# sreeramkannan/Shannon

Measured on AMD Instinct MI355X. Metric: reads/sec k-mer->graph->path-decompose, 2x100bp k=25, higher is better.
Workload: dtype u64

## Files before the change

### shannon_amd/csrc/count_sk.hip

```cpp
#include "count_views.h"
#include <algorithm>
#include <cstring>
#include <cstdlib>

#define SK_BLK 256
#define SK_RCAP 3072
#define SK_CHECK 4
#define SK_FLUSH_AT (SK_RCAP - (SK_CHECK + 1) * SK_BLK)
#define SK_TILE 32768
#define SK_CAP 2048
#ifndef SK_SCAP
#define SK_SCAP 2048
#endif
#ifndef SK_STHREADS
#define SK_STHREADS 256
#endif
#ifndef SK_T1CAP
#define SK_T1CAP 1024
#endif
#ifndef SK_T2THREADS
#define SK_T2THREADS 256
#endif
#define SK_SPILL 1280
#define SK_EMPTY 0xFFFFFFFFFFFFFFFFULL
#define SK_REGIONS 256
#define SK_RSTRIDE 16
#define SK_RANK_MAX 512
#define SK_MIN_K 20

struct SkParams { int k, m, w, bits, b1, b2; };

struct __attribute__((aligned(16))) SkRec { uint64_t hi; uint32_t lo; uint32_t meta; };

#define sk_order shn_sk_order
#define sk_bucket shn_sk_bucket

__device__ __forceinline__ void sk_extract96(const uint64_t* __restrict__ w, uint32_t nw, uint32_t p, uint64_t& hi, uint32_t& lo) {
  const uint32_t wi = p >> 5, sh = (p & 31) * 2;
  const uint64_t a = w[wi], b = wi + 1 < nw ? w[wi + 1] : 0ULL, c = (sh && wi + 2 < nw) ? w[wi + 2] : 0ULL;
  hi = sh ? (a << sh) | (b >> (64 - sh)) : a;
  const uint64_t l = sh ? (b << sh) | (c >> (64 - sh)) : b;
  lo = (uint32_t)(l >> 32);
}
__device__ __forceinline__ uint64_t sk_window(uint64_t hi, uint32_t lo, int j, int k) {
  const int sh = 2 * j;
  const uint64_t v = sh ? (hi << sh) | (((uint64_t)lo << 32) >> (64 - sh)) : hi;
  return v >> (64 - 2 * k);
}

__device__ __forceinline__ uint32_t sk_slot_hash(uint64_t key) { return (uint32_t)shn_mix64(key ^ 0x9E3779B97F4A7C15ULL); }

template <bool CANON>
__global__ __launch_bounds__(SK_BLK) void sk_scan_kernel(ReadsView v, SkParams P, uint32_t max_len, SkRec* __restrict__ slots, uint32_t S,
                                                         uint8_t* __restrict__ cnt, SkRec* __restrict__ ovf, unsigned long long* __restrict__ ovf_cursor,
                                                         uint64_t ovf_cap) {
  extern __shared__ uint32_t sk_lds[];
  uint32_t* raw = sk_lds;
  uint32_t* suf = raw + P.w * SK_BLK;
  const int tid = threadIdx.x;
  const int k = P.k, m = P.m, w = P.w;
  const uint32_t mmask = m == 16 ? 0xFFFFFFFFu : ((1u << (2 * m)) - 1u);
  const uint64_t n_tiles = (v.n_reads + SK_BLK - 1) / SK_BLK;
  for (uint64_t tile = blockIdx.x; tile < n_tiles; tile += gridDim.x) {
    const uint64_t r = tile * SK_BLK + tid;
    if (r >= v.n_reads) continue;
    const uint32_t len = v.len ? v.len[r] : v.fixed_len;
    const uint64_t wb = v.woff ? v.woff[r] : r * v.wpr;
    const uint32_t nw = v.woff ? (uint32_t)(v.woff[r + 1] - v.woff[r]) : v.wpr;
    const uint64_t* rw = v.words + wb;
    SkRec* mine = slots + r * S;
    uint64_t cur = 0, curm = 0;
    uint32_t f = 0, rr = 0, pref = 0xFFFFFFFFu, run_ord = 0, nrec = 0;
    int lastN = -1, t = 0, p0 = 0;
    bool open = false;

    auto emit = [&](int a, int b, uint32_t ord) {
      SkRec rec;
      sk_extract96(rw, nw, (uint32_t)a, rec.hi, rec.lo);
      rec.meta = (uint32_t)(b - a + 1) | (sk_bucket(ord, P.bits) << 5);
      if (nrec < S) mine[nrec] = rec;
      else {
        const unsigned long long at = atomicAdd(ovf_cursor, 1ULL);
        if (at < ovf_cap) ovf[at] = rec;
      }
      nrec++;
    };

    const uint32_t stop = len < max_len ? len : max_len;
    for (uint32_t j = 0; j < stop; j++) {
      if ((j & 31) == 0) cur = rw[j >> 5];
      const uint32_t b = (uint32_t)(cur >> (62 - 2 * (j & 31))) & 3u;
      if (v.has_n) {
        if ((j & 63) == 0) curm = v.mask[wb / 2 + (j >> 6)];
        if ((curm >> (63 - (j & 63))) & 1ULL) lastN = (int)j;
      }
      f = ((f << 2) | b) & mmask;
      rr = (rr >> 2) | ((3u - b) << (2 * (m - 1)));
      if ((int)j < m - 1) continue;
      const int i = (int)j - m + 1;
      const uint32_t ord = sk_order(CANON ? (f < rr ? f : rr) : f);
      raw[t * SK_BLK + tid] = ord;
      pref = t == 0 ? ord : (ord < pref ? ord : pref);
      if (i >= w - 1) {
        uint32_t wmin = pref;
        if (t != w - 1) { const uint32_t sv = suf[(t + 1) * SK_BLK + tid]; wmin = sv < wmin ? sv : wmin; }
        const int p = i - w + 1;
        const bool valid = lastN < p;
        if (open && (!valid || wmin != run_ord || p - p0 >= w)) { emit(p0, p - 1, run_ord); open = false; }
        if (valid && !open) { open = true; p0 = p; run_ord = wmin; }
      }
      if (t == w - 1) {
        uint32_t sm = 0xFFFFFFFFu;
        for (int tt = w - 1; tt >= 0; tt--) { const uint32_t x = raw[tt * SK_BLK + tid]; sm = x < sm ? x : sm; suf[tt * SK_BLK + tid] = sm; }
        t = 0;
      } else t++;
    }
    if (open) emit(p0, (int)len - k, run_ord);
    cnt[r] = (uint8_t)(nrec < S ? nrec : S);
  }
}

__device__ __forceinline__ bool skr_item(const SkRec* __restrict__ recs, const uint8_t* __restrict__ cnt, uint32_t S, uint64_t g, uint32_t& meta) {
  if (cnt) { const uint64_t r = g / S; if ((uint32_t)(g - r * S) >= cnt[r]) return false; }
  meta = recs[g].meta;
  return cnt || meta != 0;
}
__global__ __launch_bounds__(SK_BLK) void skr_hist_kernel(const SkRec* __restrict__ recs, const uint8_t* __restrict__ cnt, uint32_t S,
                                                          const uint64_t* __restrict__ segoff, uint32_t n_seg, int shift, uint32_t nb,
                                                          uint32_t* __restrict__ hist) {
  extern __shared__ uint32_t skh[];
  for (uint32_t p = blockIdx.y; p < n_seg; p += gridDim.y) {
    const uint64_t s0 = segoff[p], s1 = segoff[p + 1];
    const uint64_t t0 = s0 + (uint64_t)blockIdx.x * SK_TILE;
    if (t0 >= s1) continue;
    const uint64_t t1 = min(t0 + (uint64_t)SK_TILE, s1);
    for (uint32_t i = threadIdx.x; i < nb; i += SK_BLK) skh[i] = 0;
    __syncthreads();
    for (uint64_t i = t0 + threadIdx.x; i < t1; i += SK_BLK) {
      uint32_t meta;
      if (skr_item(recs, cnt, S, i, meta)) atomicAdd(&skh[((meta >> 5) >> shift) & (nb - 1)], 1u);
    }
    __syncthreads();
    for (uint32_t i = threadIdx.x; i < nb; i += SK_BLK) if (skh[i]) atomicAdd(&hist[(uint64_t)p * nb + i], skh[i]);
    __syncthreads();
  }
}
__global__ __launch_bounds__(SK_BLK) void skr_scan_rows_kernel(const uint32_t* __restrict__ hist, uint32_t nb2, uint32_t* __restrict__ off,
                                                               uint32_t* __restrict__ cursor) {
  __shared__ uint32_t part[SK_BLK];
  const uint64_t row = (uint64_t)blockIdx.x * nb2;
  const uint32_t per = (nb2 + SK_BLK - 1) / SK_BLK;
  uint32_t s = 0;
  for (uint32_t j = 0; j < per; j++) { const uint32_t i = threadIdx.x * per + j; if (i < nb2) s += hist[row + i]; }
  part[threadIdx.x] = s;
  __syncthreads();
  if (threadIdx.x == 0) { uint32_t a = 0; for (int i = 0; i < SK_BLK; i++) { const uint32_t t = part[i]; part[i] = a; a += t; } }
  __syncthreads();
  uint32_t a = part[threadIdx.x];
  for (uint32_t j = 0; j < per; j++) {
    const uint32_t i = threadIdx.x * per + j;
    if (i < nb2) { off[row + i] = a; cursor[row + i] = a; a += hist[row + i]; }
  }
}
__global__ __launch_bounds__(SK_BLK) void skr_scatter_kernel(const SkRec* __restrict__ recs, const uint8_t* __restrict__ cnt, uint32_t S,
                                                             const uint64_t* __restrict__ segoff, uint32_t n_seg, int shift, uint32_t nb,
                                                             uint32_t* __restrict__ cursor, const uint64_t* __restrict__ out_seg, SkRec* __restrict__ out) {
  extern __shared__ uint32_t sks[];
  uint32_t* lh = sks;
  uint32_t* lbase = sks + nb;
  for (uint32_t p = blockIdx.y; p < n_seg; p += gridDim.y) {
    const uint64_t s0 = segoff[p], s1 = segoff[p + 1];
    const uint64_t t0 = s0 + (uint64_t)blockIdx.x * SK_TILE;
    if (t0 >= s1) continue;
    const uint64_t t1 = min(t0 + (uint64_t)SK_TILE, s1);
    const uint64_t o0 = out_seg ? out_seg[p] : s0;
    for (uint32_t i = threadIdx.x; i < nb; i += SK_BLK) lh[i] = 0;
    __syncthreads();
    for (uint64_t i = t0 + threadIdx.x; i < t1; i += SK_BLK) {
      uint32_t meta;
      if (skr_item(recs, cnt, S, i, meta)) atomicAdd(&lh[((meta >> 5) >> shift) & (nb - 1)], 1u);
    }
    __syncthreads();
    for (uint32_t i = threadIdx.x; i < nb; i += SK_BLK) {
      const uint32_t c = lh[i];
      if (c) lbase[i] = atomicAdd(&cursor[(uint64_t)p * nb + i], c);
      lh[i] = 0;
    }
    __syncthreads();
    for (uint64_t i = t0 + threadIdx.x; i < t1; i += SK_BLK) {
      uint32_t meta;
      if (!skr_item(recs, cnt, S, i, meta)) continue;
      const SkRec rec = recs[i];
      const uint32_t q = ((meta >> 5) >> shift) & (nb - 1);
      const uint32_t rank = atomicAdd(&lh[q], 1u);
      out[o0 + lbase[q] + rank] = rec;
    }
    __syncthreads();
  }
}

template <bool CANON>
__global__ __launch_bounds__(SK_BLK) void sk_buckets_kernel(const SkRec* __restrict__ recs, const uint64_t* __restrict__ off1,
                                                            const uint32_t* __restrict__ off2, const uint32_t* __restrict__ hist2, int b2, int k, int w,
                                                            uint64_t* __restrict__ pool_keys, uint32_t* __restrict__ pool_counts,
                                                            unsigned long long* __restrict__ pool_cursor, uint64_t pool_cap) {
  constexpr int FOLD_ROUNDS_ = 2;
  __shared__ unsigned long long tk[SK_CAP];
  __shared__ uint32_t tc[SK_CAP];
  __shared__ uint32_t lnew, lpos;
  __shared__ unsigned long long lbase;
  const uint32_t b = blockIdx.x;
  const uint32_t n = hist2[b];
  if (n == 0) return;
  const uint64_t s0 = off1[b >> b2] + off2[b];
  const int tid = threadIdx.x, lane = tid & 63, q = tid & 7, grp = tid >> 3;
  for (int i = tid; i < SK_CAP; i += SK_BLK) { tk[i] = SK_EMPTY; tc[i] = 0; }
  if (tid == 0) { lnew = 0; lpos = 0; }
  __syncthreads();
  const int iters = (w + 7) >> 3;

  auto spill = [&]() {
    const uint32_t nd = lnew;
    if (tid == 0) lbase = atomicAdd(pool_cursor, (unsigned long long)nd);
    __syncthreads();
    const unsigned long long base = lbase;
    const bool fits = base + nd <= pool_cap;
    for (int i = tid; i < SK_CAP; i += SK_BLK) {
      const unsigned long long key = tk[i];
      if (key != SK_EMPTY) {
        if (fits) { const uint32_t pos = atomicAdd(&lpos, 1u); pool_keys[base + pos] = key; pool_counts[base + pos] = tc[i]; }
        tk[i] = SK_EMPTY; tc[i] = 0;
      }
    }
    __syncthreads();
    if (tid == 0) { lnew = 0; lpos = 0; }
    __syncthreads();
  };

  for (uint32_t base = 0; base < n; base += SK_BLK / 8) {
    __syncthreads();
    const bool full = lnew > SK_SPILL;
    __syncthreads();
    if (full) spill();
    const uint32_t ri = base + grp;
    SkRec rec;
    rec.hi = 0; rec.lo = 0; rec.meta = 0;
    if (ri < n) rec = recs[s0 + ri];
    const int nwin = (int)(rec.meta & 31u);
    for (int it = 0; it < iters; it++) {
      const int j = q + 8 * it;
      bool active = j < nwin;
      unsigned long long key = 0;
      if (active) {
        key = sk_window(rec.hi, rec.lo, j, k);
        if (CANON) { const uint64_t rc = shn_revcomp(key, k); key = rc < key ? rc : key; }
      }
      uint32_t wgt = active ? 1u : 0u;
      bool elect = active;
#pragma unroll
      for (int round = 0; round < FOLD_ROUNDS_; round++) {
        const unsigned long long act = __ballot(elect);
        if (!act) break;
        const int leader = __ffsll((long long)act) - 1;
        const unsigned long long lk = __shfl(key, leader, 64);
        const bool same = elect && key == lk;
        const unsigned long long msk = __ballot(same);
        if (__popcll(msk) > 1) {
          if (lane == leader) wgt = (uint32_t)__popcll(msk); else if (same) active = false;
        }
        if (same) elect = false;
      }
      if (!active) continue;
      uint32_t slot = (uint32_t)(shn_mix64(key ^ 0x9E3779B97F4A7C15ULL)) & (SK_CAP - 1);
      for (int probe = 0; probe < SK_CAP; probe++) {
        const unsigned long long prev = atomicCAS(&tk[slot], SK_EMPTY, key);
        if (prev == SK_EMPTY) { atomicAdd(&lnew, 1u); atomicAdd(&tc[slot], wgt); break; }
        if (prev == key) { atomicAdd(&tc[slot], wgt); break; }
        slot = (slot + 1) & (SK_CAP - 1);
      }
    }
  }
  __syncthreads();
  if (lnew) spill();
}

template <bool CANON, int THREADS, int CAP, int FOLD_ROUNDS_>
__global__ __launch_bounds__(THREADS) void sk_buckets_sorted_kernel(const SkRec* __restrict__ recs, const uint64_t* __restrict__ off1,
                                                                    const uint32_t* __restrict__ off2, const uint32_t* __restrict__ hist2, int b2, int k, int w,
                                                                    const uint32_t* __restrict__ list, uint32_t* __restrict__ defer, int defer_cursor,
                                                                    uint64_t* __restrict__ pool_keys, uint32_t* __restrict__ pool_counts,
                                                                    unsigned long long* __restrict__ cursors, uint64_t region_cap,
                                                                    unsigned long long* __restrict__ rcur,
                                                                    uint64_t* __restrict__ run_off, uint32_t* __restrict__ ndist) {
  extern __shared__ unsigned long long skb_lds[];
  unsigned long long* tk = skb_lds;
  uint32_t* tc = (uint32_t*)(tk + CAP);
  uint16_t* idx = (uint16_t*)(tc + CAP);
  __shared__ uint32_t lnew, lover, lpos;
  __shared__ unsigned long long lbase;
  const uint32_t b = list ? list[blockIdx.x] : blockIdx.x;
  const uint32_t n = hist2[b];
  const int tid = threadIdx.x, lane = tid & 63, q = tid & 7, grp = tid >> 3;
  if (n == 0) { if (tid == 0) { ndist[b] = 0; run_off[b] = 0; } return; }
  const uint64_t s0 = off1[b >> b2] + off2[b];
  const int iters = (w + 7) >> 3;
  const uint32_t limit = (uint32_t)(CAP - (THREADS / 8) * w - 64);

  auto pass = [&](uint32_t cls, int sbits) {
    for (int i = tid; i < CAP; i += THREADS) { tk[i] = SK_EMPTY; tc[i] = 0; }
    if (tid == 0) { lnew = 0; lover = 0; }
    __syncthreads();
    for (uint32_t base = 0; base < n; base += THREADS / 8) {
      __syncthreads();
      const bool full = lnew > limit;
      __syncthreads();
      if (full) { if (tid == 0) lover = 1; break; }
      const uint32_t ri = base + grp;
      SkRec rec;
      rec.hi = 0; rec.lo = 0; rec.meta = 0;
      if (ri < n) rec = recs[s0 + ri];
      const int nwin = (int)(rec.meta & 31u);
      for (int it = 0; it < iters; it++) {
        const int j = q + 8 * it;
        bool active = j < nwin;
        unsigned long long key = 0;
        if (active) {
          key = sk_window(rec.hi, rec.lo, j, k);
          if (CANON) { const uint64_t rc = shn_revcomp(key, k); key = rc < key ? rc : key; }
          if (sbits && (uint32_t)(key >> (2 * k - sbits)) != cls) active = false;
        }
        uint32_t wgt = active ? 1u : 0u;
        bool elect = active;
#pragma unroll
        for (int round = 0; round < FOLD_ROUNDS_; round++) {
          const unsigned long long act = __ballot(elect);
          if (!act) break;
          const int leader = __ffsll((long long)act) - 1;
          const unsigned long long lk = __shfl(key, leader, 64);
          const bool same = elect && key == lk;
          const unsigned long long msk = __ballot(same);
          if (__popcll(msk) > 1) {
            if (lane == leader) wgt = (uint32_t)__popcll(msk); else if (same) active = false;
          }
          if (same) elect = false;
        }
        if (!active) continue;
        uint32_t slot = sk_slot_hash(key) & (CAP - 1);
        for (int probe = 0; probe < CAP; probe++) {
          const unsigned long long prev = atomicCAS(&tk[slot], SK_EMPTY, key);
          if (prev == SK_EMPTY) { atomicAdd(&lnew, 1u); atomicAdd(&tc[slot], wgt); break; }
          if (prev == key) { atomicAdd(&tc[slot], wgt); break; }
          slot = (slot + 1) & (CAP - 1);
        }
      }
    }
    __syncthreads();
  };
  auto output = [&](uint64_t at) {
    const uint32_t nd = lnew;
    if (tid == 0) lpos = 0;
    __syncthreads();
    if (nd <= SK_RANK_MAX) {
      unsigned long long* dk = (unsigned long long*)idx;
      uint32_t* dc = (uint32_t*)(dk + SK_RANK_MAX);
      for (int i = tid; i < CAP; i += THREADS) {
        const unsigned long long key = tk[i];
        if (key != SK_EMPTY) { const uint32_t e = atomicAdd(&lpos, 1u); dk[e] = key; dc[e] = tc[i]; }
      }
      __syncthreads();
      for (uint32_t e = tid; e < nd; e += THREADS) {
        const unsigned long long key = dk[e];
        uint32_t r = 0;
        for (uint32_t j = 0; j < nd; j++) r += dk[j] < key ? 1u : 0u;
        pool_keys[at + r] = key; pool_counts[at + r] = dc[e];
      }
      __syncthreads();
      return;
    }
    for (int i = tid; i < CAP; i += THREADS) if (tk[i] != SK_EMPTY) idx[atomicAdd(&lpos, 1u)] = (uint16_t)i;
    uint32_t m2 = 1;
    while (m2 < nd) m2 <<= 1;
    __syncthreads();
    for (uint32_t i = nd + tid; i < m2; i += THREADS) idx[i] = 0xFFFFu;
    __syncthreads();
    for (uint32_t kk = 2; kk <= m2; kk <<= 1) {
      for (uint32_t j = kk >> 1; j > 0; j >>= 1) {
        for (uint32_t i = tid; i < m2; i += THREADS) {
          const uint32_t x = i ^ j;
          if (x > i) {
            const uint16_t ia = idx[i], ib = idx[x];
            const unsigned long long ka = ia == 0xFFFFu ? SK_EMPTY : tk[ia], kb = ib == 0xFFFFu ? SK_EMPTY : tk[ib];
            const bool asc = (i & kk) == 0;
            if ((ka > kb) == asc) { idx[i] = ib; idx[x] = ia; }
          }
        }
        __syncthreads();
      }
    }
    for (uint32_t i = tid; i < nd; i += THREADS) { const uint16_t ii = idx[i]; pool_keys[at + i] = tk[ii]; pool_counts[at + i] = tc[ii]; }
    __syncthreads();
  };

  int sbits = 0;
  uint32_t total = 0;
  for (;;) {
    total = 0;
    bool ok = true;
    for (uint32_t cls = 0; cls < (1u << sbits); cls++) {
      pass(cls, sbits);
      if (lover) { ok = false; break; }
      total += lnew;
      if (sbits == 0) break;
      __syncthreads();
    }
    if (ok) break;
    if (defer) {
      if (tid == 0) { const unsigned long long at = atomicAdd(&cursors[defer_cursor], 1ULL); defer[at] = b; ndist[b] = 0; run_off[b] = 0; }
      return;
    }
    sbits += 2;
    if (sbits > 16 || sbits > 2 * k) {
      if (tid == 0) { atomicAdd(&cursors[3], 1ULL); ndist[b] = 0; run_off[b] = 0; }
      return;
    }
    __syncthreads();
  }
  const uint32_t reg = b & (SK_REGIONS - 1);
  if (tid == 0) lbase = atomicAdd(&rcur[reg * SK_RSTRIDE], (unsigned long long)total);
  __syncthreads();
  const unsigned long long in_reg = lbase, base = (unsigned long long)reg * region_cap + in_reg;
  if (in_reg + total > region_cap) { if (tid == 0) { ndist[b] = 0; run_off[b] = 0; } return; }
  if (tid == 0) { ndist[b] = total; run_off[b] = base; }
  if (sbits == 0) { output(base); return; }
  uint64_t at = base;
  for (uint32_t cls = 0; cls < (1u << sbits); cls++) {
    pass(cls, sbits);
    const uint32_t nd = lnew;
    output(at);
    at += nd;
  }
}
__global__ __launch_bounds__(SK_BLK) void sk_gather_kernel(const uint64_t* __restrict__ pool_keys, const uint32_t* __restrict__ pool_counts,
                                                           const uint64_t* __restrict__ run_off, const uint32_t* __restrict__ ndist,
                                                           const uint64_t* __restrict__ boff, uint64_t n_buckets, uint64_t* __restrict__ keys,
                                                           uint32_t* __restrict__ counts) {
  const uint64_t b = ((uint64_t)blockIdx.x * SK_BLK + threadIdx.x) / SHN_WAVE;
  if (b >= n_buckets) return;
  const uint32_t lane = threadIdx.x & (SHN_WAVE - 1);
  const uint32_t nd = ndist[b];
  const uint64_t s0 = run_off[b], d0 = boff[b];
  for (uint32_t i = lane; i < nd; i += SHN_WAVE) { keys[d0 + i] = pool_keys[s0 + i]; counts[d0 + i] = pool_counts[s0 + i]; }
}
__global__ void sk_sum_counts_kernel(const uint32_t* __restrict__ c, uint64_t n, unsigned long long* __restrict__ out) {
  unsigned long long a = 0;
  for (uint64_t i = (uint64_t)blockIdx.x * blockDim.x + threadIdx.x; i < n; i += (uint64_t)gridDim.x * blockDim.x) a += c[i];
  for (int o = 32; o > 0; o >>= 1) a += __shfl_down(a, o, 64);
  if ((threadIdx.x & 63) == 0 && a) atomicAdd(out, a);
}

int shn_count_superkmers(shn_ctx* ctx, const std::vector<ReadsView>& views, uint64_t upper, int k1, int both_strands, shn_table** out, int* handled) {
  *handled = 0;
  const int mode = (int)shn_env_u64("SHN_COUNT_SK", 1);
  if (mode == 0 || k1 < SK_MIN_K || (k1 == 32 && !both_strands) || upper == 0) return SHN_OK;
  if (mode != 2 && upper < (1ULL << 22)) return SHN_OK;
  hipStream_t s = ctx->stream; shn_use_stream(s);
  SkParams P;
  P.k = k1;
  P.m = std::max(13, 2 * k1 - 48);
  P.w = k1 - P.m + 1;
  int bits = 6;
  while (bits < 22 && (upper >> bits) > 3500) bits++;
  bits = (int)shn_env_u64("SHN_COUNT_SK_BITS", (uint64_t)bits, 4, 22);
  P.bits = bits;
  P.b1 = (bits + 1) / 2;
  P.b2 = bits - P.b1;
  const uint32_t nb1 = 1u << P.b1, nb2 = 1u << P.b2;
  const uint64_t nbk = 1ULL << bits;
  struct ViewPlan { uint64_t slot0, read0; uint32_t S, max_len; };
  std::vector<ViewPlan> plan(views.size());
  uint64_t n_slots = 0, n_reads = 0;
  for (size_t i = 0; i < views.size(); i++) {
    const ReadsView& v = views[i];
    const double expect = 2.0 * v.wmax / (P.w + 1) + 1.0;
    uint32_t S = ((uint32_t)(expect * 1.35 + 1.999) + 3u) & ~3u;
    S = std::max<uint32_t>(1, std::min<uint32_t>(std::min<uint32_t>(S, 252), std::max<uint32_t>(v.wmax, 1)));
    S = (uint32_t)shn_env_u64("SHN_COUNT_SK_SLOTS", S, 1, 252);
    plan[i] = ViewPlan{n_slots, n_reads, S, v.wmax ? v.wmax + (uint32_t)k1 - 1 : 0u};
    if (v.wmax && v.n_reads) { n_slots += v.n_reads * S; n_reads += v.n_reads; }
  }
  const uint64_t ovf_cap = n_reads / 2 + 4096;
  int rc;
  void *p, *pslots, *pcnt;
  const size_t small = (size_t)nb1 * 4 * 3 + 64 + ((size_t)nb1 + 4) * 8 + nbk * 4 * 3 + 64 + (views.size() + 2) * 16;
  if ((rc = shn_ws(ctx)[22].get(small, &p))) return rc;
  if ((rc = shn_ws(ctx)[18].get((n_slots + ovf_cap + 2) * sizeof(SkRec), &pslots))) return rc;
  if ((rc = shn_ws(ctx)[23].get(n_reads + 64, &pcnt))) return rc;
  uint32_t* d_hist1 = (uint32_t*)p;
  uint32_t* d_offr1 = d_hist1 + nb1;
  uint32_t* d_cursor1 = d_offr1 + nb1;
  unsigned long long* d_cursors = (unsigned long long*)(d_cursor1 + nb1 + ((nb1 & 1) ? 1 : 0));
  uint64_t* d_seg = (uint64_t*)(d_cursors + 8);
  uint32_t* d_hist2 = (uint32_t*)(d_seg + nb1 + 4);
  uint32_t* d_off2 = d_hist2 + nbk;
  uint32_t* d_cursor2 = d_off2 + nbk;
  uint64_t* d_pairs = (uint64_t*)(d_cursor2 + nbk + (nbk & 1));
  SkRec* slots = (SkRec*)pslots;
  SkRec* ovf = slots + n_slots;
  uint8_t* d_cnt = (uint8_t*)pcnt;
  HIP_TRY(hipMemsetAsync(d_hist1, 0, (size_t)nb1 * 4, s));
  HIP_TRY(hipMemsetAsync(d_cursors, 0, 64, s));
  HIP_TRY(hipMemsetAsync(ovf, 0, ovf_cap * sizeof(SkRec), s));
  const size_t lds_scan = (size_t)2 * P.w * SK_BLK * 4;
  for (size_t i = 0; i < views.size(); i++) {
    const ReadsView& v = views[i];
    if (!v.wmax || !v.n_reads) continue;
    TimerRegion t(ctx, T_SK_EMIT);
    const uint32_t grid = (uint32_t)std::min<uint64_t>(cdiv(v.n_reads, SK_BLK), 1u << 20);
    if (both_strands) hipLaunchKernelGGL(sk_scan_kernel<true>, dim3(grid), dim3(SK_BLK), lds_scan, s, v, P, plan[i].max_len, slots + plan[i].slot0, plan[i].S,
                                         d_cnt + plan[i].read0, ovf, d_cursors, ovf_cap);
    else hipLaunchKernelGGL(sk_scan_kernel<false>, dim3(grid), dim3(SK_BLK), lds_scan, s, v, P, plan[i].max_len, slots + plan[i].slot0, plan[i].S,
                            d_cnt + plan[i].read0, ovf, d_cursors, ovf_cap);
  }
  std::vector<uint64_t> pairs(2 * (views.size() + 1), 0);
  for (size_t i = 0; i <= views.size(); i++) pairs[2 * i + 1] = i == views.size() ? ovf_cap : ((views[i].wmax && views[i].n_reads) ? views[i].n_reads * plan[i].S : 0);
  HIP_TRY(hipMemcpyAsync(d_pairs, pairs.data(), pairs.size() * 8, hipMemcpyHostToDevice, s));
  auto level1 = [&](bool scatter, SkRec* recsA) {
    for (size_t i = 0; i <= views.size(); i++) {
      const bool is_ovf = i == views.size();
      const uint64_t n = pairs[2 * i + 1];
      if (!n) continue;
      const SkRec* in = is_ovf ? ovf : slots + plan[i].slot0;
      const uint8_t* c = is_ovf ? nullptr : d_cnt + plan[i].read0;
      const uint32_t S = is_ovf ? 1u : plan[i].S;
      const uint32_t tiles = (uint32_t)std::max<uint64_t>(1, cdiv(n, SK_TILE));
      if (!scatter) hipLaunchKernelGGL(skr_hist_kernel, dim3(tiles, 1), dim3(SK_BLK), nb1 * 4, s, in, c, S, d_pairs + 2 * i, 1u, P.b2, nb1, d_hist1);
      else hipLaunchKernelGGL(skr_scatter_kernel, dim3(tiles, 1), dim3(SK_BLK), nb1 * 8, s, in, c, S, d_pairs + 2 * i, 1u, P.b2, nb1, d_cursor1,
                              (const uint64_t*)(d_cursors + 4), recsA);
    }
  };
  {
    TimerRegion t(ctx, T_SK_HIST);
    level1(false, nullptr);
  }
  std::vector<uint32_t> h1(nb1);
  unsigned long long ovf_used = 0;
  HIP_TRY(hipMemcpyAsync(h1.data(), d_hist1, (size_t)nb1 * 4, hipMemcpyDeviceToHost, s));
  HIP_TRY(hipMemcpyAsync(&ovf_used, d_cursors, 8, hipMemcpyDeviceToHost, s));
  HIP_TRY(hipStreamSynchronize(s));
  HIP_TRY(hipGetLastError());
  if (ovf_used > ovf_cap) return SHN_OK;
  std::vector<uint64_t> off1(nb1 + 1);
  std::vector<uint32_t> off1r(nb1);
  uint64_t NR = 0, max1 = 0;
  for (uint32_t i = 0; i < nb1; i++) { off1[i] = NR; NR += h1[i]; max1 = std::max<uint64_t>(max1, h1[i]); }
  off1[nb1] = NR;
  if (NR >= 0xFFFFFFFFULL) return SHN_OK;
  for (uint32_t i = 0; i < nb1; i++) off1r[i] = (uint32_t)off1[i];
  void* pa;
  if ((rc = shn_ws(ctx)[19].get((NR + 2) * sizeof(SkRec), &pa))) return rc;
  SkRec* recsA = (SkRec*)pa;
  SkRec* recsB = slots;
  HIP_TRY(hipMemcpyAsync(d_cursor1, off1r.data(), (size_t)nb1 * 4, hipMemcpyHostToDevice, s));
  HIP_TRY(hipMemcpyAsync(d_seg, off1.data(), (size_t)(nb1 + 1) * 8, hipMemcpyHostToDevice, s));
  HIP_TRY(hipMemsetAsync(d_hist2, 0, nbk * 4, s));
  HIP_TRY(hipStreamSynchronize(s));
  {
    TimerRegion t(ctx, T_SK_HIST);
    level1(true, recsA);
  }
  const uint32_t tiles = (uint32_t)std::max<uint64_t>(1, cdiv(max1, SK_TILE));
  {
    TimerRegion t(ctx, T_SK_HIST2);
    hipLaunchKernelGGL(skr_hist_kernel, dim3(tiles, nb1), dim3(SK_BLK), nb2 * 4, s, recsA, (const uint8_t*)nullptr, 1u, d_seg, nb1, 0, nb2, d_hist2);
  }
  hipLaunchKernelGGL(skr_scan_rows_kernel, dim3(nb1), dim3(SK_BLK), 0, s, d_hist2, nb2, d_off2, d_cursor2);
  {
    TimerRegion t(ctx, T_SK_SCATTER2);
    hipLaunchKernelGGL(skr_scatter_kernel, dim3(tiles, nb1), dim3(SK_BLK), nb2 * 8, s, recsA, (const uint8_t*)nullptr, 1u, d_seg, nb1, 0, nb2, d_cursor2,
                       (const uint64_t*)nullptr, recsB);
  }
  double ratio = ctx->sk_pool_ratio > 0 ? ctx->sk_pool_ratio * 1.05 : 0.125;
  ratio = shn_env_double("SHN_COUNT_SK_POOL", ratio);
  uint64_t cap = std::min<uint64_t>(upper, (uint64_t)((double)upper * ratio) + 4096);
  uint64_t np = 0;
  void *pk = nullptr, *pc = nullptr;
  bool sorted = shn_env_u64("SHN_COUNT_SK_LAYOUT", 1) != 0;
  if (sorted) {
    void* pr;
    if ((rc = shn_ws(ctx)[24].get(nbk * 20 + 64, &pr))) return rc;
    uint64_t* d_run_off = (uint64_t*)pr;
    uint32_t* d_ndist = (uint32_t*)(d_run_off + nbk);
    uint32_t* d_defer = d_ndist + nbk;
    uint32_t* d_defer2 = d_defer + nbk;
    constexpr int T1_CAP = SK_T1CAP, T2_CAP = SK_SCAP, BIG_T = 1024, BIG_CAP = 8192;
    const size_t lds_t1 = (size_t)T1_CAP * 12 + std::max<size_t>((size_t)T1_CAP * 2, (size_t)SK_RANK_MAX * 12),
                 lds_t2 = (size_t)T2_CAP * 12 + std::max<size_t>((size_t)T2_CAP * 2, (size_t)SK_RANK_MAX * 12), lds_big = (size_t)BIG_CAP * 14;
    HIP_TRY(hipFuncSetAttribute((const void*)sk_buckets_sorted_kernel<true, BIG_T, BIG_CAP, 2>, hipFuncAttributeMaxDynamicSharedMemorySize, (int)lds_big));
    HIP_TRY(hipFuncSetAttribute((const void*)sk_buckets_sorted_kernel<false, BIG_T, BIG_CAP, 2>, hipFuncAttributeMaxDynamicSharedMemorySize, (int)lds_big));
    unsigned long long cur[8] = {0, 0, 0, 0, 0, 0, 0, 0};
    void* prc;
    if ((rc = shn_ws(ctx)[29].get((size_t)SK_REGIONS * SK_RSTRIDE * 8, &prc))) return rc;
    unsigned long long* d_rcur = (unsigned long long*)prc;
    std::vector<unsigned long long> h_rcur((size_t)SK_REGIONS * SK_RSTRIDE);
    for (int attempt = 0; attempt < 3 && sorted; attempt++) {
      const uint64_t region_cap = cap / SK_REGIONS + 64;
      if ((rc = shn_ws(ctx)[20].get((region_cap * SK_REGIONS + 2) * 8, &pk))) return rc;
      if ((rc = shn_ws(ctx)[21].get((region_cap * SK_REGIONS + 2) * 4, &pc))) return rc;
      HIP_TRY(hipMemsetAsync(d_cursors + 1, 0, 56, s));
      HIP_TRY(hipMemsetAsync(d_rcur, 0, (size_t)SK_REGIONS * SK_RSTRIDE * 8, s));
      {
#define SK_LAUNCH(CANON_, T_, CAP_, FOLD_, GRID_, LDS_, LIST_, DEFER_, DCUR_) \
        hipLaunchKernelGGL((sk_buckets_sorted_kernel<CANON_, T_, CAP_, FOLD_>), dim3((uint32_t)(GRID_)), dim3(T_), LDS_, s, recsB, d_seg, d_off2, d_hist2, P.b2, k1, P.w, \
                           (const uint32_t*)(LIST_), (uint32_t*)(DEFER_), DCUR_, (uint64_t*)pk, (uint32_t*)pc, d_cursors, region_cap, d_rcur, d_run_off, d_ndist)
        { TimerRegion t(ctx, T_SK_BUCKETS);
          if (both_strands) SK_LAUNCH(true, SK_STHREADS, T1_CAP, 0, nbk, lds_t1, nullptr, d_defer, 2);
          else SK_LAUNCH(false, SK_STHREADS, T1_CAP, 0, nbk, lds_t1, nullptr, d_defer, 2); }
        HIP_TRY(hipMemcpyAsync(cur, d_cursors, 64, hipMemcpyDeviceToHost, s));
        HIP_TRY(hipStreamSynchronize(s));
        const unsigned long long n_t2 = cur[2];
        if (n_t2) {
          TimerRegion t2(ctx, T_SK_BUCKETS2);
          if (both_strands) SK_LAUNCH(true, SK_T2THREADS, T2_CAP, 0, n_t2, lds_t2, d_defer, d_defer2, 6);
          else SK_LAUNCH(false, SK_T2THREADS, T2_CAP, 0, n_t2, lds_t2, d_defer, d_defer2, 6);
          HIP_TRY(hipMemcpyAsync(cur, d_cursors, 64, hipMemcpyDeviceToHost, s));
          HIP_TRY(hipStreamSynchronize(s));
        }
        if (shn_env_set("SHN_COUNT_SK_DEBUG")) fprintf(stderr, "[sk] buckets %llu, %llu of them to 2,048 slots, %llu to 8,192; pool of %llu pairs in %d stretches\n", (unsigned long long)nbk, n_t2, cur[6], (unsigned long long)cap, SK_REGIONS);
        if (cur[6]) {
          TimerRegion tb(ctx, T_SK_BIG);
          if (both_strands) SK_LAUNCH(true, BIG_T, BIG_CAP, 2, cur[6], lds_big, d_defer2, nullptr, 2);
          else SK_LAUNCH(false, BIG_T, BIG_CAP, 2, cur[6], lds_big, d_defer2, nullptr, 2);
          HIP_TRY(hipMemcpyAsync(cur, d_cursors, 64, hipMemcpyDeviceToHost, s));
          HIP_TRY(hipStreamSynchronize(s));
        }
#undef SK_LAUNCH
      }
      HIP_TRY(hipGetLastError());
      if (cur[3]) { sorted = false; break; }
      HIP_TRY(hipMemcpyAsync(h_rcur.data(), d_rcur, h_rcur.size() * 8, hipMemcpyDeviceToHost, s));
      HIP_TRY(hipStreamSynchronize(s));
      unsigned long long fullest = 0;
      np = 0;
      for (int r_ = 0; r_ < SK_REGIONS; r_++) { const unsigned long long u = h_rcur[(size_t)r_ * SK_RSTRIDE]; np += u; fullest = std::max(fullest, u); }
      if (fullest <= region_cap) break;
      if (attempt == 2) return shn_fail(SHN_ERR_OVERFLOW, "shn_count_k1mers: the pair pool of the super-k-mer path stayed too small");
      cap = std::max<uint64_t>(np + np / 64 + 4096, (fullest + fullest / 64 + 64) * SK_REGIONS);
    }
    if (sorted) {
      if (!shn_env_set("SHN_COUNT_SK_POOL")) ctx->sk_pool_ratio = (double)np / (double)upper;
      shn_table* t = new shn_table();
      memset(t, 0, sizeof(*t));
      t->ctx = ctx; t->device = ctx->device; t->k = k1; t->canonical = both_strands ? 1 : 0; t->bits = bits; t->n_buckets = nbk;
      t->layout = 1; t->sk_m = P.m; t->n = np;
#define TRYT(x) do { hipError_t _e = (x); if (_e != hipSuccess) { shn_table_destroy(t); return shn_fail(SHN_ERR_HIP, std::string(#x) + ": " + hipGetErrorString(_e)); } } while (0)
      TRYT(shn_dev_malloc(&t->d_keys, (np + 1) * 8));
      TRYT(shn_dev_malloc(&t->d_counts, (np + 1) * 4));
      TRYT(shn_dev_malloc(&t->d_bucket_off, (nbk + 1) * 8));
      uint64_t D = 0;
      { TimerRegion tr(ctx, T_COMPACT);
        if ((rc = shn_device_scan_u32(ctx, d_ndist, nbk, t->d_bucket_off, &D))) { shn_table_destroy(t); return rc; }
        if (D != np) { shn_table_destroy(t); return shn_fail(SHN_ERR_OVERFLOW, "shn_count_k1mers: super-k-mer buckets and pool disagree"); }
        if (np) hipLaunchKernelGGL(sk_gather_kernel, dim3((uint32_t)cdiv(nbk * SHN_WAVE, SK_BLK)), dim3(SK_BLK), 0, s, (const uint64_t*)pk, (const uint32_t*)pc,
                                   (const uint64_t*)d_run_off, (const uint32_t*)d_ndist, (const uint64_t*)t->d_bucket_off, nbk, t->d_keys, t->d_counts);
        TRYT(hipMemsetAsync(d_cursors + 5, 0, 8, s));
        if (np) hipLaunchKernelGGL(sk_sum_counts_kernel, dim3(1024), dim3(256), 0, s, (const uint32_t*)t->d_counts, np, d_cursors + 5);
        unsigned long long tot = 0;
        TRYT(hipMemcpyAsync(&tot, d_cursors + 5, 8, hipMemcpyDeviceToHost, s));
        TRYT(hipStreamSynchronize(s));
        TRYT(hipGetLastError());
        t->total = tot;
      }
#undef TRYT
      *out = t;
      *handled = 1;
      return SHN_OK;
    }
  }
  for (int attempt = 0; attempt < 3; attempt++) {
    if ((rc = shn_ws(ctx)[20].get((cap + 2) * 8, &pk))) return rc;
    if ((rc = shn_ws(ctx)[21].get((cap + 2) * 4, &pc))) return rc;
    HIP_TRY(hipMemsetAsync(d_cursors + 1, 0, 8, s));
    {
      TimerRegion t(ctx, T_SK_BUCKETS);
      if (both_strands) hipLaunchKernelGGL(sk_buckets_kernel<true>, dim3((uint32_t)nbk), dim3(SK_BLK), 0, s, recsB, d_seg, d_off2, d_hist2, P.b2, k1, P.w,
                                           (uint64_t*)pk, (uint32_t*)pc, d_cursors + 1, cap);
      else hipLaunchKernelGGL(sk_buckets_kernel<false>, dim3((uint32_t)nbk), dim3(SK_BLK), 0, s, recsB, d_seg, d_off2, d_hist2, P.b2, k1, P.w,
                              (uint64_t*)pk, (uint32_t*)pc, d_cursors + 1, cap);
    }
    unsigned long long used = 0;
    HIP_TRY(hipMemcpyAsync(&used, d_cursors + 1, 8, hipMemcpyDeviceToHost, s));
    HIP_TRY(hipStreamSynchronize(s));
    HIP_TRY(hipGetLastError());
    np = used;
    if (np <= cap) break;
    if (attempt == 2) return shn_fail(SHN_ERR_OVERFLOW, "shn_count_k1mers: the pair pool of the super-k-mer path stayed too small");
    cap = std::min<uint64_t>(upper, np + np / 64 + 4096);
  }
  if (np >= 0xFFFFFFFFULL) return SHN_OK;
  rc = shn_table_from_pairs(ctx, pk, pc, np, k1, both_strands ? 1 : 0, out);
  if (rc) return rc;
  HIP_TRY(hipStreamSynchronize(s));
  *handled = 1;
  return SHN_OK;
}
```

Measured before the change: 66.75 million.

## Load-balance super-k-mer windows across threads and pre-route large buckets to deferred tiers

The bucket counting kernel now spreads windows evenly over threads. It stages one record per thread in LDS, takes a block prefix sum of window counts, and has each thread binary-search its start record. Before, each 8-thread group handled one record, which wasted lanes on short records. Buckets with more records than a threshold now skip straight to the deferred list, so they are not half-counted in the small table, and the next record is prefetched while the current round runs. The cost is extra syncs, a binary search, more LDS and a new routing parameter, plus a debug histogram.

```diff
diff --git a/shannon_amd/csrc/count_sk.hip b/shannon_amd/csrc/count_sk.hip
--- a/shannon_amd/csrc/count_sk.hip
+++ b/shannon_amd/csrc/count_sk.hip
@@ -26,6 +26,12 @@
 #define SK_REGIONS 256
 #define SK_RSTRIDE 16
 #define SK_RANK_MAX 512
+#ifndef SK_ROUTE1
+#define SK_ROUTE1 1536u
+#endif
+#ifndef SK_ROUTE2
+#define SK_ROUTE2 0xFFFFFFFFu
+#endif
 #define SK_MIN_K 20
 
 struct SkParams { int k, m, w, bits, b1, b2; };
@@ -287,45 +293,80 @@
 template <bool CANON, int THREADS, int CAP, int FOLD_ROUNDS_>
 __global__ __launch_bounds__(THREADS) void sk_buckets_sorted_kernel(const SkRec* __restrict__ recs, const uint64_t* __restrict__ off1,
                                                                     const uint32_t* __restrict__ off2, const uint32_t* __restrict__ hist2, int b2, int k, int w,
-                                                                    const uint32_t* __restrict__ list, uint32_t* __restrict__ defer, int defer_cursor,
+                                                                    const uint32_t* __restrict__ list, uint32_t* __restrict__ defer, int defer_cursor, uint32_t route,
                                                                     uint64_t* __restrict__ pool_keys, uint32_t* __restrict__ pool_counts,
                                                                     unsigned long long* __restrict__ cursors, uint64_t region_cap,
                                                                     unsigned long long* __restrict__ rcur,
                                                                     uint64_t* __restrict__ run_off, uint32_t* __restrict__ ndist) {
-  extern __shared__ unsigned long long skb_lds[];
+  static_assert(CAP > THREADS + 64 && THREADS % 64 == 0, "a round of THREADS windows must fit the table");
+  extern __shared__ __attribute__((aligned(16))) unsigned long long skb_lds[];
   unsigned long long* tk = skb_lds;
   uint32_t* tc = (uint32_t*)(tk + CAP);
   uint16_t* idx = (uint16_t*)(tc + CAP);
+  SkRec* stage = (SkRec*)idx;
+  uint32_t* wend = (uint32_t*)(stage + THREADS);
   __shared__ uint32_t lnew, lover, lpos;
+  __shared__ uint32_t wsum[THREADS / 64];
   __shared__ unsigned long long lbase;
   const uint32_t b = list ? list[blockIdx.x] : blockIdx.x;
   const uint32_t n = hist2[b];
-  const int tid = threadIdx.x, lane = tid & 63, q = tid & 7, grp = tid >> 3;
+  const uint64_t o1 = off1[b >> b2];
+  const uint32_t o2 = off2[b];
+  const int tid = threadIdx.x, lane = tid & 63;
   if (n == 0) { if (tid == 0) { ndist[b] = 0; run_off[b] = 0; } return; }
-  const uint64_t s0 = off1[b >> b2] + off2[b];
-  const int iters = (w + 7) >> 3;
-  const uint32_t limit = (uint32_t)(CAP - (THREADS / 8) * w - 64);
+  if (defer && n > route) {
+    if (tid == 0) { const unsigned long long at = atomicAdd(&cursors[defer_cursor], 1ULL); defer[at] = b; ndist[b] = 0; run_off[b] = 0; }
+    return;
+  }
+  const uint64_t s0 = o1 + o2;
+  const uint32_t limit = (uint32_t)(CAP - THREADS - 64);
 
   auto pass = [&](uint32_t cls, int sbits) {
+    SkRec nxt;
+    nxt.hi = 0; nxt.lo = 0; nxt.meta = 0;
+    if ((uint32_t)tid < n) nxt = recs[s0 + tid];
     for (int i = tid; i < CAP; i += THREADS) { tk[i] = SK_EMPTY; tc[i] = 0; }
     if (tid == 0) { lnew = 0; lover = 0; }
-    __syncthreads();
-    for (uint32_t base = 0; base < n; base += THREADS / 8) {
+    uint32_t bound = 0;
+    bool over = false;
+    for (uint32_t base = 0; base < n && !over; base += THREADS) {
+      const SkRec rec = nxt;
+      uint32_t inc = rec.meta & 31u;
+      for (int o = 1; o < 64; o <<= 1) { const uint32_t y = __shfl_up(inc, o, 64); if (lane >= o) inc += y; }
       __syncthreads();
-      const bool full = lnew > limit;
+      stage[tid] = rec;
+      if (lane == 63) wsum[tid >> 6] = inc;
       __syncthreads();
-      if (full) { if (tid == 0) lover = 1; break; }
-      const uint32_t ri = base + grp;
-      SkRec rec;
-      rec.hi = 0; rec.lo = 0; rec.meta = 0;
-      if (ri < n) rec = recs[s0 + ri];
-      const int nwin = (int)(rec.meta & 31u);
-      for (int it = 0; it < iters; it++) {
-        const int j = q + 8 * it;
-        bool active = j < nwin;
+      uint32_t pre = 0, W = 0;
+      for (int i = 0; i < THREADS / 64; i++) { const uint32_t x = wsum[i]; pre += i < (tid >> 6) ? x : 0u; W += x; }
+      wend[tid] = pre + inc;
+      nxt.hi = 0; nxt.lo = 0; nxt.meta = 0;
+      if (base + THREADS + (uint32_t)tid < n) nxt = recs[s0 + base + THREADS + tid];
+      __syncthreads();
+      const uint32_t c = (W + THREADS - 1) / THREADS;
+      const uint32_t g = (uint32_t)tid * c;
+      uint32_t r = 0;
+      if (g < W) {
+        uint32_t lo_ = 0, hi_ = THREADS - 1;
+        while (lo_ < hi_) { const uint32_t mid = (lo_ + hi_) >> 1; if (wend[mid] > g) hi_ = mid; else lo_ = mid + 1; }
+        r = lo_;
+      }
+      SkRec cur = stage[r];
+      uint32_t nwr = cur.meta & 31u;
+      uint32_t j = g < W ? g - (wend[r] - nwr) : 0u;
+      for (uint32_t i = 0; i < c; i++) {
+        if (bound > limit) {
+          __syncthreads();
+          bound = lnew;
+          __syncthreads();
+          if (bound > limit) { if (tid == 0) lover = 1; over = true; break; }
+        }
+        bound += THREADS;
+        bool active = g + i < W;
+        const bool mine = active;
         unsigned long long key = 0;
         if (active) {
-          key = sk_window(rec.hi, rec.lo, j, k);
+          key = sk_window(cur.hi, cur.lo, (int)j, k);
           if (CANON) { const uint64_t rc = shn_revcomp(key, k); key = rc < key ? rc : key; }
           if (sbits && (uint32_t)(key >> (2 * k - sbits)) != cls) active = false;
         }
@@ -344,13 +385,18 @@
           }
           if (same) elect = false;
         }
-        if (!active) continue;
-        uint32_t slot = sk_slot_hash(key) & (CAP - 1);
-        for (int probe = 0; probe < CAP; probe++) {
-          const unsigned long long prev = atomicCAS(&tk[slot], SK_EMPTY, key);
-          if (prev == SK_EMPTY) { atomicAdd(&lnew, 1u); atomicAdd(&tc[slot], wgt); break; }
-          if (prev == key) { atomicAdd(&tc[slot], wgt); break; }
-          slot = (slot + 1) & (CAP - 1);
+        if (active) {
+          uint32_t slot = sk_slot_hash(key) & (CAP - 1);
+          for (int probe = 0; probe < CAP; probe++) {
+            const unsigned long long prev = atomicCAS(&tk[slot], SK_EMPTY, key);
+            if (prev == SK_EMPTY) { atomicAdd(&lnew, 1u); atomicAdd(&tc[slot], wgt); break; }
+            if (prev == key) { atomicAdd(&tc[slot], wgt); break; }
+            slot = (slot + 1) & (CAP - 1);
+          }
+        }
+        if (mine && ++j == nwr && g + i + 1 < W) {
+          do { r++; cur = stage[r]; nwr = cur.meta & 31u; } while (nwr == 0 && r < THREADS - 1);
+          j = 0;
         }
       }
     }
@@ -593,8 +639,10 @@
     uint32_t* d_defer = d_ndist + nbk;
     uint32_t* d_defer2 = d_defer + nbk;
     constexpr int T1_CAP = SK_T1CAP, T2_CAP = SK_SCAP, BIG_T = 1024, BIG_CAP = 8192;
-    const size_t lds_t1 = (size_t)T1_CAP * 12 + std::max<size_t>((size_t)T1_CAP * 2, (size_t)SK_RANK_MAX * 12),
-                 lds_t2 = (size_t)T2_CAP * 12 + std::max<size_t>((size_t)T2_CAP * 2, (size_t)SK_RANK_MAX * 12), lds_big = (size_t)BIG_CAP * 14;
+    auto lds_of = [](size_t cap_, size_t threads) { return cap_ * 12 + std::max<size_t>(std::max<size_t>(cap_ * 2, (size_t)SK_RANK_MAX * 12), threads * 20); };
+    const size_t lds_t1 = lds_of(T1_CAP, SK_STHREADS), lds_t2 = lds_of(T2_CAP, SK_T2THREADS), lds_big = lds_of(BIG_CAP, BIG_T);
+    const bool sk_debug = shn_env_set("SHN_COUNT_SK_DEBUG");
+    const uint32_t route1 = sk_debug ? 0xFFFFFFFFu : SK_ROUTE1, route2 = sk_debug ? 0xFFFFFFFFu : SK_ROUTE2;
     HIP_TRY(hipFuncSetAttribute((const void*)sk_buckets_sorted_kernel<true, BIG_T, BIG_CAP, 2>, hipFuncAttributeMaxDynamicSharedMemorySize, (int)lds_big));
     HIP_TRY(hipFuncSetAttribute((const void*)sk_buckets_sorted_kernel<false, BIG_T, BIG_CAP, 2>, hipFuncAttributeMaxDynamicSharedMemorySize, (int)lds_big));
     unsigned long long cur[8] = {0, 0, 0, 0, 0, 0, 0, 0};
@@ -609,27 +657,44 @@
       HIP_TRY(hipMemsetAsync(d_cursors + 1, 0, 56, s));
       HIP_TRY(hipMemsetAsync(d_rcur, 0, (size_t)SK_REGIONS * SK_RSTRIDE * 8, s));
       {
-#define SK_LAUNCH(CANON_, T_, CAP_, FOLD_, GRID_, LDS_, LIST_, DEFER_, DCUR_) \
+#define SK_LAUNCH(CANON_, T_, CAP_, FOLD_, GRID_, LDS_, LIST_, DEFER_, DCUR_, ROUTE_) \
         hipLaunchKernelGGL((sk_buckets_sorted_kernel<CANON_, T_, CAP_, FOLD_>), dim3((uint32_t)(GRID_)), dim3(T_), LDS_, s, recsB, d_seg, d_off2, d_hist2, P.b2, k1, P.w, \
-                           (const uint32_t*)(LIST_), (uint32_t*)(DEFER_), DCUR_, (uint64_t*)pk, (uint32_t*)pc, d_cursors, region_cap, d_rcur, d_run_off, d_ndist)
+                           (const uint32_t*)(LIST_), (uint32_t*)(DEFER_), DCUR_, ROUTE_, (uint64_t*)pk, (uint32_t*)pc, d_cursors, region_cap, d_rcur, d_run_off, d_ndist)
         { TimerRegion t(ctx, T_SK_BUCKETS);
-          if (both_strands) SK_LAUNCH(true, SK_STHREADS, T1_CAP, 0, nbk, lds_t1, nullptr, d_defer, 2);
-          else SK_LAUNCH(false, SK_STHREADS, T1_CAP, 0, nbk, lds_t1, nullptr, d_defer, 2); }
+          if (both_strands) SK_LAUNCH(true, SK_STHREADS, T1_CAP, 0, nbk, lds_t1, nullptr, d_defer, 2, route1);
+          else SK_LAUNCH(false, SK_STHREADS, T1_CAP, 0, nbk, lds_t1, nullptr, d_defer, 2, route1); }
         HIP_TRY(hipMemcpyAsync(cur, d_cursors, 64, hipMemcpyDeviceToHost, s));
         HIP_TRY(hipStreamSynchronize(s));
         const unsigned long long n_t2 = cur[2];
         if (n_t2) {
           TimerRegion t2(ctx, T_SK_BUCKETS2);
-          if (both_strands) SK_LAUNCH(true, SK_T2THREADS, T2_CAP, 0, n_t2, lds_t2, d_defer, d_defer2, 6);
-          else SK_LAUNCH(false, SK_T2THREADS, T2_CAP, 0, n_t2, lds_t2, d_defer, d_defer2, 6);
+          if (both_strands) SK_LAUNCH(true, SK_T2THREADS, T2_CAP, 0, n_t2, lds_t2, d_defer, d_defer2, 6, route2);
+          else SK_LAUNCH(false, SK_T2THREADS, T2_CAP, 0, n_t2, lds_t2, d_defer, d_defer2, 6, route2);
           HIP_TRY(hipMemcpyAsync(cur, d_cursors, 64, hipMemcpyDeviceToHost, s));
           HIP_TRY(hipStreamSynchronize(s));
         }
-        if (shn_env_set("SHN_COUNT_SK_DEBUG")) fprintf(stderr, "[sk] buckets %llu, %llu of them to 2,048 slots, %llu to 8,192; pool of %llu pairs in %d stretches\n", (unsigned long long)nbk, n_t2, cur[6], (unsigned long long)cap, SK_REGIONS);
+        if (sk_debug) {
+          fprintf(stderr, "[sk] buckets %llu, %llu of them to 2,048 slots, %llu to 8,192; pool of %llu pairs in %d stretches\n", (unsigned long long)nbk, n_t2, cur[6], (unsigned long long)cap, SK_REGIONS);
+          std::vector<uint32_t> h2(nbk), l1(n_t2), l2(cur[6]);
+          HIP_TRY(hipMemcpy(h2.data(), d_hist2, nbk * 4, hipMemcpyDeviceToHost));
+          if (n_t2) HIP_TRY(hipMemcpy(l1.data(), d_defer, n_t2 * 4, hipMemcpyDeviceToHost));
+          if (cur[6]) HIP_TRY(hipMemcpy(l2.data(), d_defer2, cur[6] * 4, hipMemcpyDeviceToHost));
+          constexpr uint32_t STEP = 64, NBIN = 256;
+          std::vector<uint64_t> all(NBIN, 0), f1(NBIN, 0), f2(NBIN, 0);
+          auto bin = [&](uint32_t n_) { return std::min<uint32_t>(n_ ? (n_ - 1) / STEP : 0, NBIN - 1); };
+          for (uint64_t i = 0; i < nbk; i++) all[bin(h2[i])]++;
+          for (uint32_t b_ : l1) f1[bin(h2[b_])]++;
+          for (uint32_t b_ : l2) f2[bin(h2[b_])]++;
+          uint64_t ca = 0, c1 = 0, c2 = 0;
+          for (int i = NBIN - 1; i >= 0; i--) {
+            ca += all[i]; c1 += f1[i]; c2 += f2[i];
+            if (all[i]) fprintf(stderr, "[sk] records > %u: %llu buckets, %llu filled 1,024 slots, %llu filled 2,048\n", i * STEP, (unsigned long long)ca, (unsigned long long)c1, (unsigned long long)c2);
+          }
+        }
         if (cur[6]) {
           TimerRegion tb(ctx, T_SK_BIG);
-          if (both_strands) SK_LAUNCH(true, BIG_T, BIG_CAP, 2, cur[6], lds_big, d_defer2, nullptr, 2);
-          else SK_LAUNCH(false, BIG_T, BIG_CAP, 2, cur[6], lds_big, d_defer2, nullptr, 2);
+          if (both_strands) SK_LAUNCH(true, BIG_T, BIG_CAP, 2, cur[6], lds_big, d_defer2, nullptr, 2, 0xFFFFFFFFu);
+          else SK_LAUNCH(false, BIG_T, BIG_CAP, 2, cur[6], lds_big, d_defer2, nullptr, 2, 0xFFFFFFFFu);
           HIP_TRY(hipMemcpyAsync(cur, d_cursors, 64, hipMemcpyDeviceToHost, s));
           HIP_TRY(hipStreamSynchronize(s));
         }
```

New measurement: 66.10 million. About the same (-1.0%).
